# MarineRoboticsGroup/score

Hardware: AMD Instinct MI355X
Metric: socp_iters_per_sec (higher is better)
Workload: dtype f64; 1 GPU; BASELINE configs[3]: manhattan RA-SLAM, 20 robots x 1000 poses, 4 beacons, SOCP relaxation, 1 trial(s)/GPU, ADMM loop alone (polish off) to eps 1e-07; n=146995, m=80979, nnz_P=946147, parallelism=independent x1

## Files before the change

### score_amd/csrc/score_hip.hip

```cpp
#include <hip/hip_runtime.h>
#include <sched.h>
#include <sys/prctl.h>
#include <time.h>
#include <hip/hip_ext.h>

#include <cstdio>
#include <cstring>
#include <malloc.h>
#include <mutex>
#include <string>
#include <memory>
#include <optional>
#include <vector>

#include "score_driver.hpp"
#include <future>
#include "score_assemble.hpp"
#include "score_gn_kernels.hpp"
#include "score_round.hpp"
#include "score_kernels.hpp"
#include "score_polish.hpp"
#include "score_polish_device.hpp"
#include "score_setup_device.hpp"
#include "score_prec_wave.hpp"
// ... 511 lines not shown
        total = 0;
    }
};

inline bool long_spin_enabled() {
    static const bool on = std::getenv("SCORE_NO_LONG_SPIN") == nullptr;
    return on;
}

struct CsrBufs {
    DevBuf<int32_t> ptr, col, first_row, blk_prob, blk_rs, split;
    DevBuf<int4> blk_meta, blk_long;
    DevBuf<double> long_part;
    DevBuf<unsigned long long> long_cnt;
    void alloc_long(int n_long, int n_slots) {
        long_part.alloc((size_t)std::max(1, n_slots) * kLongVals);
        long_cnt.alloc((size_t)std::max(1, n_long));
        fill_zero_async(long_cnt.d, long_cnt.n * sizeof(unsigned long long), tl_copy_stream);
        fill_words_async(long_part.d, (uint32_t)kLongSentinel32, long_part.n * sizeof(double), tl_copy_stream);
    }
    int spin_max_tiles = 0;
    DevBuf<double> val;
    int nblocks = 0;
    int rep = 1;
    int unroll = kUnroll;
    int rs_in = 0;
    void adopt_tiles(const Csr& M, const RowBlocks& rb) {
        UploadBatch ub;
        first_row.upload(rb.first_row);
        blk_prob.upload(rb.prob);
        blk_rs.upload(rb.rs);
// ... 60 lines not shown
        nblocks = L.nb();
        UploadBatch ub;
        V.alloc((size_t)L.v_size + 64);
        fill_zero_async(V.d, V.n * sizeof(double), tl_copy_stream);
        rem_col.upload_padded(L.rem_col, 64);
        rowseg.upload(L.rowseg); dst.upload(L.dst); prob.upload(L.prob); rs.upload(L.rs); part_ptr.upload(L.part_ptr);
        std::vector<int4> m((size_t)nblocks), m2((size_t)nblocks);
        for (int b = 0; b < nblocks; ++b) {
            m[(size_t)b] = make_int4(L.meta[4 * (size_t)b], L.meta[4 * (size_t)b + 1], L.meta[4 * (size_t)b + 2], L.meta[4 * (size_t)b + 3]);
            m2[(size_t)b] = make_int4(L.meta2[4 * (size_t)b], L.meta2[4 * (size_t)b + 1], L.meta2[4 * (size_t)b + 2], L.meta2[4 * (size_t)b + 3]);
        }
        meta.upload(m); meta2.upload(m2);
        std::vector<int4> lg((size_t)nblocks);
        for (int b = 0; b < nblocks; ++b) lg[(size_t)b] = make_int4(L.lng[4 * (size_t)b], L.lng[4 * (size_t)b + 1], L.lng[4 * (size_t)b + 2], L.lng[4 * (size_t)b + 3]);
        lng.upload(lg);
        long_part.alloc((size_t)std::max(1, L.n_long_slots) * kLongVals);
        long_cnt.alloc((size_t)std::max(1, L.n_long));
        fill_zero_async(long_cnt.d, long_cnt.n * sizeof(unsigned long long), tl_copy_stream);
        fill_words_async(long_part.d, (uint32_t)kLongSentinel32, long_part.n * sizeof(double), tl_copy_stream);
    }
    BandDev dev() const {
        BandDev d{};
        d.val = V.d; d.rem_col = rem_col.d; d.rowseg = rowseg.d; d.meta2 = meta2.d; d.rem0 = (int32_t)L.rem0; d.bs = L.bs;
        for (int j = 0; j < kBandMaxS / 2; ++j) d.offw[j] = L.offw[j];
        return d;
    }
};

struct RuizDevice : RuizOffload {
    int device = 0;
    DevArena keep;
// ... 123 lines not shown
        return std::getenv("SCORE_NO_BAND") == nullptr;
    }
    DevBuf<int32_t> A_ptr, A_col;
    DevBuf<double> A_val;
    DevBuf<double> q, b, invD, invE, rho, K0d, K1d;
    DevBuf<int32_t> done, cone_row, cone_dim, cone_type, cone_block_first, cone_block_prob;
    DevBuf<int4> cone_meta;
    DevBuf<int2> cone_large;
    int n_large_cones = 0;
    DevBuf<int32_t> cone_cols;
    DevBuf<double> cone_vals;
    DevBuf<int32_t> node_col, diag_cols, prec_part_ptr;
    DevBuf<PrecWork> prec_work, factor_work;
    DevBuf<int64_t> q_entpart;
    int64_t q_ent_max = 0;
    static constexpr int64_t kHelpEntries = (int64_t)kPrecThreads * kPrecChunk;
    int n_help = 0;
    DevBuf<int32_t> vb_first, vb_end, vb_prob;
    int n_vblocks = 0;
    DevBuf<double> xtu, xy, s, r, z, p, p2, w, kx, step;
    DevBuf<double> pw_part, rz_part0, rz_part1, rz_meas0, rz_meas1, pres_part, dres_part;
    struct GenSource {
        const int32_t* rel_base; const int32_t* rel_to; const double* rel_t; const double* rel_R; const double* rel_kappa; const double* rel_tau;
        const int32_t* rng_a; const int32_t* rng_b; const double* rng_dist; const double* rng_prec;
    };
    const GenSource* gen_src = nullptr;
    int n_join_items = 0, n_join_chains = 0, n_join_seps = 0;
    DevBuf<JoinChain> join_jc;
    DevBuf<JoinItem> join_items;
    DevBuf<int32_t> join_sep_col, join_sep_diag, join_pcol, join_pprev, join_zero;
// ... 775 lines not shown
        }
        set_replica_strides(h);
        upload_cone_tables(h);
        pt.mark("  uploads: cone records");
        {
            UploadBatch ub_tables;
            upload_chain_tables(h);
            plan_split_kernel(h);
        }
        pt.mark("uploads");
        plan_chain_kernel(h);
        const bool polish_from_device = st.polish && init_polish_build(h);
        pt.mark("polish: structure (before the band view is waited for)");
        adopt_band_view(h, pt);
        carve_iterates(h);
        cg_iters = st.cg_iters;
        done.upload(std::vector<int32_t>((size_t)h.count, 0));
        upload_k0_k1(h);
        chain_positions(h);
        join_init(h);
        alloc_factors(h);
        pt.mark("allocations + rho data (device)");
        if (st.polish) init_polish(h, polish_from_device);
        link_init(h, probs, graphs);
        pt.mark("polish setup");
        carve_report_and_control(h);
        reset();
        pt.mark("reset");
        drain_setup();
        pt.mark("staged uploads: drain");
// ... 261 lines not shown
        pl.pre_lds = pl.pre ? lds_pre : 0;
        pl.reg = pl.pre && h.deep_ok && h.bs <= 3 && st.fac_fp32 != 0;
        pl.reg_lds = pl.reg ? lds_reg : 0;
        return pl;
    }
    void plan_chain_kernel(const HostSystem& h) {
        const ChainKernelPlan pl = chain_kernel_plan(h);
        prec_lds0 = pl.lds0; prec_lds = pl.lds;
        prec_pre = pl.pre; prec_pre_lds = pl.pre_lds;
        prec_reg = pl.reg; prec_reg_lds = pl.reg_lds;
        if (prec_reg) deep_map.upload(h.deep_map);
        const bool fallback = !prec_pre || (h.bs >= 4 && st.fac_fp32 == 0);
        if (fallback && prec_lds > 144 * 1024) throw std::runtime_error("chain too long: more than 129 segments of 1023 nodes (132 k) for the segmented chain solver, and beyond what the streaming kernel keeps in LDS");
        if (n_prec_chains(h)) with_bs([&](auto bs) { allow_big_lds<decltype(bs)::value>(); });
    }
    void adopt_band_view(HostSystem& h, PhaseTimer& pt) {
        if (band_job.valid()) {
            Kb.upload(band_job.get());
            if (Kb.on)
                for (int p = 0; p < h.count; ++p) h.kkt_bytes[(size_t)p] = Kb.L.bytes[(size_t)p] + 16.0 * (double)(h.xoff[p + 1] - h.xoff[p]);
            if (st.verbose)
                std::fprintf(stderr, "[score setup] band view of K: %s (%d band + %d csr + %d diag tiles, %d slots per row)\n", Kb.on ? "on" : "off",
                             Kb.L.n_band, Kb.L.n_csr, Kb.L.n_diag, Kb.L.S);
            pt.mark("band view of K (wait + upload)");
        }
        Kset.blk_part.upload(Kb.on ? Kb.L.part_ptr : h.rbK.part_ptr);
    }
    void carve_iterates(const HostSystem& h) {
        const size_t nm = (size_t)(h.n_tot + h.m_tot), nn = (size_t)h.n_tot, mm = (size_t)h.m_tot, cc = (size_t)h.count;
        const size_t kb = (size_t)Kset.blocks(), np_ = (size_t)n_prec;
// ... 625 lines not shown

    SpmvArgs spmv_args(const CsrBufs& M, const double* xin) {
        SpmvArgs a{};
        a.M = M.dev(); a.xin = xin; a.done = done.d; a.rs_in = M.rs_in;
        a.n_tiles = M.nblocks;
        a.x = xy.d; a.q = q.d; a.kx = kx.d; a.r = r.d; a.sigma = H->sigma;
        a.p = p.d; a.w = w.d; a.pw_part = pw_part.d;
        a.prec_part_ptr = prec_part_ptr.d; a.kblk_part_ptr = Kset.blk_part.d;
        a.uni = uni_for(Kset.blocks());
        a.apply_update = 0; a.pfin = p.d; a.wfin = w.d; a.xt_rw = xtu.d; a.kx_rw = kx.d; a.x_rw = xy.d;
        a.alpha_relax = st.alpha; a.step_in = step.d;
        a.invD = invD.d; a.dres_part = dres_part.d;
        return a;
    }

    void launch_kp(const double* pdir, unsigned long long* ts = nullptr, int slot = -1) {
        SpmvArgs a = spmv_args(K, pdir);
        a.p = pdir; a.tstamp = ts;
        launch_product<MODE_KP>(Kset, a, slot);
    }
    void launch_kpb(const double* p_old, double* p_new, const double* rz_new, const double* rz_old,
                    unsigned long long* ts = nullptr, int slot = -1) {
        SpmvArgs a = spmv_args(K, p_old);
        a.tstamp = ts;
        a.p = p_old; a.z = z.d; a.p_out = p_new; a.rz_new = rz_new; a.rz_old = rz_old;
        launch_product<MODE_KPB>(Kset, a, slot);
    }

    void set_cg_iters(int k) {
        cg_iters = std::max(1, k);
        if (graph_exec) { (void)hipGraphExecDestroy(graph_exec); graph_exec = nullptr; }
    }

// ... 10 lines not shown
        }
    }

    VecArgs xupdate_args(const double* p_dir, const double* rz_old, int apply_alpha) {
        VecArgs va{};
        va.first_row = vb_first.d; va.end_row = vb_end.d; va.blk_prob = vb_prob.d; va.done = done.d;
        va.prec_part_ptr = prec_part_ptr.d; va.kblk_part_ptr = Kset.blk_part.d;
        va.pw_part = pw_part.d; va.p = p_dir; va.w = w.d; va.kx = kx.d; va.xt = xtu.d; va.x = xy.d;
        va.alpha_relax = st.alpha; va.rz_old = rz_old; va.apply_alpha = apply_alpha;
        return va;
    }

    size_t ts_stride = 0;
    void enqueue_iteration(bool measure, bool first, unsigned long long* ts = nullptr) {
        auto slot = [&](int k) -> unsigned long long* { return ts ? ts + ts_stride * k : nullptr; };
        {
            SpmvArgs ra = spmv_args(G1, xtu.d);
            ra.tstamp = slot(0);
            ra.apply_update = first ? 0 : 1;
            ra.pfin = last_p;
            launch_spmv<MODE_RHS>(G1, ra, 0);
        }
        PrecArgs pa = prec_args(Kset);
        pa.done = done.d;
        prec_vectors(pa, r.d, r.d, z.d, p.d, w.d, xtu.d, kx.d, pw_part.d);
        double* rz_cur = measure ? rz_meas0.d : rz_part0.d;
        double* p_cur = p.d;
        double* p_oth = p2.d;
        pa.p = p_cur; pa.rz_in = nullptr; pa.rz_out = rz_cur;
        pa.tstamp = slot(1);
        launch_prec<PREC_INIT>(Kset, pa, 1);
        launch_kp(p_cur, slot(2), 2);
        for (int j = 2; j <= cg_iters; ++j) {
            double* rz_nxt = (rz_cur == rz_part0.d) ? rz_part1.d : rz_part0.d;
            pa.p = p_cur; pa.rz_in = rz_cur; pa.rz_out = rz_nxt;
            pa.tstamp = (j == 2) ? slot(3) : nullptr;
            launch_prec<PREC_STEP>(Kset, pa, (j == 2) ? 3 : -1);
            launch_kpb(p_cur, p_oth, rz_nxt, rz_cur, (j == 2) ? slot(4) : nullptr, (j == 2) ? 4 : -1);
            std::swap(p_cur, p_oth);
            rz_cur = rz_nxt;
        }
        dbg_p = p_cur;
        ConeArgs ca = cone_args(xtu.d);
        if (measure) {
            pa.tstamp = nullptr;
            pa.p = p_cur; pa.rz_in = rz_cur; pa.rz_out = rz_meas1.d;
            launch_prec<PREC_STEP>(Kset, pa);
            hipLaunchKernelGGL(k_xupdate, dim3(n_vblocks), dim3(kThreads), 0, stream, xupdate_args(p_cur, rz_cur, 0));
        } else {
            ca.apply_alpha = 1; ca.pfin = p_cur; ca.rz_in = rz_cur;
            last_rz = rz_cur;
            last_p = p_cur;
        }
        ca.tstamp = slot(5);
        if (n_cone_blocks) {
            int chunk = 0;
            const unsigned cgrid = xcd_grid_of(n_cone_blocks, chunk);
            if (chunk) { ca.xcd_chunk = chunk; ca.n_blocks = n_cone_blocks; }
            launch_on_stream(k_cone, dim3(cgrid), dim3(kThreads), 0, 5, ca);
            ca.xcd_chunk = 0;
// ... 1413 lines not shown
```

### score_amd/csrc/score_inspect.hpp

```cpp
#pragma once

struct NewtonProbe {
    static constexpr int kCap = 1024;
    bool armed = false;
    std::vector<hipEvent_t> ev;
    struct Slot { int kind, step; bool real; };
    std::vector<Slot> slots;
    size_t marked = 0;
    double out[8] = {0, 0, 0, 0, 0, 0, 0, 0};
};
int probe_slot(HipBackend& be, int kind, int step) {
    NewtonProbe* np = be.probe.get();
    if (!np || !np->armed || (int)np->slots.size() >= NewtonProbe::kCap) return -1;
    np->slots.push_back(NewtonProbe::Slot{kind, step, false});
    be.tev = np->ev.data();
    return (int)np->slots.size() - 1;
}
void probe_mark(HipBackend& be, int used) {
    NewtonProbe* np = be.probe.get();
    if (!np) return;
    for (; np->marked < np->slots.size(); ++np->marked)
        if (np->slots[np->marked].step < used) np->slots[np->marked].real = true;
}
void probe_collect(HipBackend& be) {
// ... 101 lines not shown
    return copy_out_min(v, 3, out, len);
}
int64_t get_links(HipBackend& be, double* out, int64_t len) {
    double v[6] = {(double)be.link_plan.pairs_total, (double)be.link_plan.pairs_used, (double)be.n_link_u, (double)be.n_link_items, (double)be.link_rounds, 0.0};
    if (be.n_link_probs && out) {
        std::vector<int32_t> stt((size_t)be.n_link_probs);
        HIP_CHECK(sync_stream(be.stream));
        for (int set = 0; set < 2; ++set) {
            if (!be.pset[set].link_on) continue;
            HIP_CHECK(hipMemcpy(stt.data(), be.pset[set].link_status.d, sizeof(int32_t) * (size_t)be.n_link_probs, hipMemcpyDeviceToHost));
            for (int32_t x : stt) v[5] += x;
        }
    }
    return copy_out_min(v, 6, out, len);
}
int64_t get_newton_probe(HipBackend& be, double* out, int64_t len) {
    static const double none[8] = {0, 0, 0, 0, 0, 0, 0, 0};
    return copy_out_min(be.probe ? be.probe->out : none, 8, out, len);
}
double mismatches(const std::vector<int32_t>& x, const std::vector<int32_t>& y) {
    double c = (double)(x.size() > y.size() ? x.size() - y.size() : y.size() - x.size());
    for (size_t i = 0; i < std::min(x.size(), y.size()); ++i) c += x[i] != y[i];
    return c;
}
double max_diff(const std::vector<double>& x, const std::vector<double>& y) {
    double c = x.size() == y.size() ? 0.0 : 1e300;
    for (size_t i = 0; i < std::min(x.size(), y.size()); ++i) c = std::max(c, std::fabs(x[i] - y[i]));
    return c;
}
int64_t get_ag_device_check(HipBackend& be, double* out, int64_t len) {
// ... 105 lines not shown
        {"is_head", ds ? R::DevI32 : R::HostI32, ds ? (const void*)be.q_ishead.d : Q.is_head.data(), ds ? n : (int64_t)Q.is_head.size(), polish},
        {"Hcol", be.polish_on_device ? R::DevI32 : R::HostI32, be.polish_on_device ? (const void*)be.Hm.col.d : Q.Hm.col.data(),
         be.polish_on_device ? be.hm_nnz : (int64_t)Q.Hm.col.size(), polish},
        {"Hptr", R::HostI32, Q.Hm.ptr.data(), (int64_t)Q.Hm.ptr.size(), polish},
        {"link_pairs", R::HostI32, be.link_plan.pair_cols.data(), be.n_link_items ? (int64_t)be.link_plan.pair_cols.size() : 0},
    };
    for (const R& r : rows)
        if (nm == r.name) return read_row(be, r, out, len);
    struct Computed { const char* name; int64_t (*fn)(HipBackend&, double*, int64_t); };
    static const Computed computed[] = {
        {"setup_scalars", get_setup_scalars}, {"device_setup", get_device_setup}, {"rep", get_rep}, {"links", get_links},
        {"newton_probe_arm", probe_arm}, {"newton_probe", get_newton_probe}, {"ag_device_check", get_ag_device_check},
        {"polish_build_check", get_polish_build_check}, {"polish_assemble_at_x", get_polish_assemble_at_x},
        {"polish_prec_of_negg", get_polish_prec_of_negg},
        {"chain_of_col", get_chain_of_col}, {"chain_id_of_col", get_chain_id_of_col}, {"matrix_source", get_matrix_source},
    };
    for (const Computed& c : computed)
        if (nm == c.name) return c.fn(be, out, len);
    return -1;
}

struct TimeAllActive {
    HipBackend& be;
    std::vector<int32_t> keep;
    explicit TimeAllActive(HipBackend& b) : be(b), keep((size_t)b.H->count) {
        const std::vector<int32_t> zero(keep.size(), 0);
        HIP_CHECK(sync_stream(be.stream));
        HIP_CHECK(hipMemcpyAsync(keep.data(), be.done.d, keep.size() * sizeof(int32_t), hipMemcpyDeviceToHost, be.stream));
        HIP_CHECK(sync_stream(be.stream));
        HIP_CHECK(hipMemcpyAsync(be.done.d, zero.data(), zero.size() * sizeof(int32_t), hipMemcpyHostToDevice, be.stream));
// ... 128 lines not shown
```

### score_amd/csrc/score_kernels.hpp

```cpp
#pragma once

#include <type_traits>

#include <hip/hip_runtime.h>

#include "score_host.hpp"
#include "score_band.hpp"

namespace score {

#ifdef SCORE_NT_STORES
#define NTS(lhs, val) __builtin_nontemporal_store((val), &(lhs))
#else
#define NTS(lhs, val) ((lhs) = (val))
#endif
#if defined(SCORE_NT_STORES) || defined(SCORE_NT_PREC)
#define NTSP(lhs, val) __builtin_nontemporal_store((val), &(lhs))
#else
#define NTSP(lhs, val) ((lhs) = (val))
#endif

constexpr int kThreads = 256;
constexpr int kUnroll = kTileNnz / kThreads;
constexpr int kLongUnroll = 2;
constexpr int kPartStride = 12;

__device__ __forceinline__ double wave_sum(double v) {
#pragma unroll
    for (int off = 32; off > 0; off >>= 1) v += __shfl_down(v, off, 64);
    return v;
}
__device__ __forceinline__ double wave_max(double v) {
#pragma unroll
    for (int off = 32; off > 0; off >>= 1) v = fmax(v, __shfl_down(v, off, 64));
    return v;
}
__device__ __forceinline__ double block_sum(double v, double* red) {
    v = wave_sum(v);
    __syncthreads();
    if ((threadIdx.x & 63) == 0) red[threadIdx.x >> 6] = v;
// ... 53 lines not shown

struct CsrDev {
    const int32_t* ptr;
    const int32_t* col;
    const double* val;
    const int32_t* first_row;
    const int32_t* blk_prob;
    const int4* blk_meta;
    const int32_t* blk_rs;
    const int32_t* split;
    int nblocks;
    const int4* blk_long;
    double* long_part;
    unsigned long long* long_cnt;
    int long_spin;
};
constexpr unsigned long long kLongSentinel = 0x7ff8dead7ff8deadull;
constexpr unsigned kLongSentinel32 = 0x7ff8deadu;

struct KernelStamp {
    unsigned long long* ts;
    __device__ explicit KernelStamp(unsigned long long* p) : ts(p) {
        if (ts && threadIdx.x == 0) ts[2 * blockIdx.x] = (unsigned long long)wall_clock64();
    }
    __device__ ~KernelStamp() {
        if (ts && threadIdx.x == 0) ts[2 * blockIdx.x + 1] = (unsigned long long)wall_clock64();
    }
};

struct UniRanges {
    int on;
    int l0, l1;
    int k0, k1;
};

struct BandDev {
    const double* val;
    const int32_t* rem_col;
    const int32_t* rowseg;
    const int4* meta2;
    int32_t rem0;
    int32_t bs;
    int32_t offw[kBandMaxS / 2];
};

struct SpmvArgs {
    UniRanges uni;
    CsrDev M;
    BandDev B;
// ... 22 lines not shown
    double* xt_rw;
    double* kx_rw;
    double* x_rw;
    double alpha_relax;
    const double* step_in;
    const int32_t* kblk_part_ptr;
    const int32_t* is_head;
    double* gout;
    const double* invD;
    double* dres_part;
    unsigned long long* tstamp;
};

enum { MODE_RHS = 0, MODE_KP = 1, MODE_DRES = 2, MODE_KPB = 3, MODE_GRAD = 4 };

constexpr int kMaxRep = 3;

__device__ __forceinline__ void soc_scales(int type, double t0, double nz2, double& head, double& tail) {
    if (type == 0) {
        head = 0.0; tail = 0.0;
        return;
    }
    const double nz = sqrt(nz2);
    if (nz <= t0) { head = t0; tail = 1.0; }
    else if (nz <= -t0) { head = 0.0; tail = 0.0; }
    else { const double m = 0.5 * (t0 + nz); head = m; tail = m / nz; }
}

struct TileHead {
    int4 meta, m2, lg;
    int prob, rs, dn0;
};
// ... 45 lines not shown
        if (MODE == MODE_KPB) {
            if (pi0 < pl1) { acc_n = a.rz_new[pi0]; acc_o = a.rz_old[pi0]; }
            for (int i = pi0 + kThreads; i < pl1; i += kThreads) { acc_n += a.rz_new[i]; acc_o += a.rz_old[i]; }
        }
    };
    if (MODE == MODE_RHS && a.apply_update) beta = a.step_in[prob];
    auto finish_beta = [&]() {
        if (MODE == MODE_KPB) {
            block_sum2(acc_n, acc_o, red);
            beta = acc_o > 0.0 ? acc_n / acc_o : 0.0;
        }
    };

    int row = r0 + t;
    bool has_row = false;
    double sum[NR], sum2 = 0.0;
#pragma unroll
    for (int q = 0; q < NR; ++q) sum[q] = 0.0;
    const int dn = a.uni.on ? dn0 : a.done[prob];
    const int my_ptr = a.M.ptr[min(r0 + t, r1)];
    const int nseg = lg.y & 0xffff;
    const bool one_long = (r1 - r0 == 1 && (nn > kLongRow || nseg > 1));
    int b = b_in;
    const int ro = one_long ? r0 : min(row, max(r1 - 1, r0));
    double e0[NR], e1[NR], e2[NR], e3[NR], e4[NR], e5[NR];
#pragma unroll
    for (int q = 0; q < NR; ++q) {
        const int o = ro + q * rs_out;
        e0[q] = e1[q] = e2[q] = e3[q] = e4[q] = e5[q] = 0.0;
        if (MODE == MODE_RHS) {
// ... 62 lines not shown
                    if ((MODE == MODE_DRES || MODE == MODE_GRAD) && k >= split) acc2 += pr; else acc[q] += pr;
                }
            }
        }
        if (MODE == MODE_DRES || MODE == MODE_GRAD) {
            block_sum2(acc[0], acc2, red);
            sum[0] = acc[0]; sum2 = acc2;
        } else if (NR == 1) {
            sum[0] = block_sum(acc[0], red);
        } else {
            block_sum2(acc[0], acc[1], red);
            sum[0] = acc[0]; sum[1] = acc[1];
            if (NR > 2) sum[NR - 1] = block_sum(acc[NR - 1], red);
        }
        const bool spin = nseg > 1 && a.M.long_spin && nseg * kLongVals <= NR * kPlane;
        if (spin) {
            constexpr int NV = NR + ((MODE == MODE_DRES || MODE == MODE_GRAD) ? 1 : 0);
            const int sgi = lg.y >> 16;
            unsigned long long* allb = reinterpret_cast<unsigned long long*>(a.M.long_part + (size_t)lg.z * kLongVals);
            if (sgi != 0) {
                if (t == 0) {
                    unsigned long long* slot = allb + (size_t)sgi * kLongVals;
#pragma unroll
                    for (int q = 0; q < NR; ++q) __hip_atomic_store(slot + q, (unsigned long long)__double_as_longlong(sum[q]), __ATOMIC_RELAXED, __HIP_MEMORY_SCOPE_AGENT);
                    if (MODE == MODE_DRES || MODE == MODE_GRAD)
                        __hip_atomic_store(slot + NR, (unsigned long long)__double_as_longlong(sum2), __ATOMIC_RELAXED, __HIP_MEMORY_SCOPE_AGENT);
                }
                return;
            }
            const int total = nseg * kLongVals;
            int ok = 0;
// ... 129 lines not shown
    if (MODE == MODE_RHS) {
        if (has_row) {
#pragma unroll
            for (int q = 0; q < NR; ++q) {
                const int o = row + q * rs_out;
                double kxv = e0[q];
                double xv = e1[q];
                if (a.apply_update) {
                    const double xt = e3[q] + beta * e4[q];
                    kxv += beta * e5[q];
                    xv = a.alpha_relax * xt + (1.0 - a.alpha_relax) * xv;
                    NTS(a.xt_rw[o], xt);
                    NTS(a.kx_rw[o], kxv);
                    NTS(a.x_rw[o], xv);
                }
                NTS(a.r[o], a.sigma * xv - e2[q] + sum[q] - kxv);
            }
        }
    } else if (MODE == MODE_KP || MODE == MODE_KPB) {
        double local = 0.0;
        if (has_row) {
#pragma unroll
            for (int q = 0; q < NR; ++q) {
                const int o = row + q * rs_out;
                double pi, sq = sum[q];
                if (MODE == MODE_KPB) {
                    sq += beta * e0[q];
                    pi = e1[q] + beta * e2[q];
                    NTS(a.p_out[o], pi);
                } else {
                    pi = e0[q];
// ... 352 lines not shown
struct PrecArgs {
    const PrecWork* work;
    const PrecRecord* rec;
    const ChainDesc* chains;
    const ChainLevelDesc* levels;
    const double* fac;
    const float* fac32;
    const float* deep;
    const int32_t* node_col;
    const int32_t* diag_cols;
    const double* dinv;
    const int32_t* done;
    const int32_t* prec_part_ptr;
    const int32_t* kblk_part_ptr;
    UniRanges uni;
    double* r;
    double* z;
    double* p;
    const double* w;
    double* xt;
    double* kx;
    const double* rz_in;
    const double* pw_part;
    double* rz_out;
    unsigned long long* tstamp;
    int debug_skip;
    int n_vec;
    long long vec_stride;
    int split_update;
    const double* r_in;
// ... 55 lines not shown
    const size_t eP = (size_t)L.P * L.nruns;
    const double* __restrict__ R = fac + L.offR;
#pragma unroll
    for (int q = 0; q < RMAX; ++q) {
        const double* __restrict__ Rq = R + (size_t)min(q, len - 1) * L.nruns + j;
#pragma unroll
        for (int e = 0; e < B2; ++e) {
            Lf[q][e] = Rq[(size_t)e * eP];
            Dv[q][e] = Rq[(size_t)(B2 + e) * eP];
        }
    }
}

template <int MODE>
__device__ __forceinline__ double prec_jacobi_item(const PrecArgs& a, const PrecWork& wk, double acc_rz, double acc_pw,
                                                   double* red, bool& stop) {
    const int t = threadIdx.x;
    double alpha = 0.0, local = 0.0;
    stop = false;
    if (MODE == PREC_STEP) {
        const double gref = (a.gate_flag && !a.gate_first) ? a.gate_ref[wk.prob] : 0.0;
        block_sum2_n<kPrecWaves>(acc_rz, acc_pw, red);
        alpha = acc_pw > 0.0 ? acc_rz / acc_pw : 0.0;
        if (pcg_gate(a, wk.prob, acc_rz, gref)) { stop = true; return 0.0; }
    }
    const int e_end = wk.index + wk.count;
    for (int base = wk.index + t; base < e_end; base += kPrecThreads * kPrecChunk) {
        int cols[kPrecChunk];
        double rv[kPrecChunk], dv[kPrecChunk], pv[kPrecChunk], wv[kPrecChunk], xv[kPrecChunk], kv[kPrecChunk];
#pragma unroll
        for (int u = 0; u < kPrecChunk; ++u) cols[u] = a.diag_cols[min(base + u * kPrecThreads, e_end - 1)];
#pragma unroll
        for (int u = 0; u < kPrecChunk; ++u) {
            rv[u] = a.r_in[cols[u]];
            dv[u] = a.dinv[min(base + u * kPrecThreads, e_end - 1)];
            if (MODE == PREC_STEP) {
                wv[u] = a.w[cols[u]];
                if (!a.split_update) { pv[u] = a.p[cols[u]]; xv[u] = a.xt_zero ? 0.0 : a.xt[cols[u]]; kv[u] = a.kx[cols[u]]; }
                else { pv[u] = 0.0; xv[u] = 0.0; kv[u] = 0.0; }
            }
        }
#pragma unroll
        for (int u = 0; u < kPrecChunk; ++u) {
            if (base + u * kPrecThreads < e_end) {
                double r_ = rv[u];
                if (MODE == PREC_STEP) {
                    if (!a.split_update) {
                        NTSP(a.xt[cols[u]], xv[u] + alpha * pv[u]);
                        NTSP(a.kx[cols[u]], kv[u] + alpha * wv[u]);
                    }
                    r_ -= alpha * wv[u];
                    NTSP(a.r[cols[u]], r_);
                }
                const double zv = r_ * dv[u];
                NTSP(a.z[cols[u]], zv);
                if (MODE == PREC_INIT) NTSP(a.p[cols[u]], zv);
                local += r_ * zv;
            }
        }
    }
    return local;
}

__device__ __forceinline__ void prec_select_vector(PrecArgs& a) {
    if (a.n_vec > 1) {
        const long long off = (long long)blockIdx.y * a.vec_stride;
// ... 334 lines not shown
    constexpr int B2 = BS * BS;
    constexpr int oRun = REGDEEP ? 2 * B2 : 0;
    constexpr int oBk2 = 10 * B2;
    constexpr int NG = REGDEEP ? 12 * B2 : PreTile<BS>::NG;
    constexpr int oCl = oRun + 2 * RMAX * B2, oCr = oCl + B2;
    constexpr int kStageLanes = kPrecThreads - kPreRunLanes;
    constexpr int CH = PreTile<BS>::CH;
    using LT = typename std::conditional<(BS >= 4 || REGDEEP), FT, double>::type;
    extern __shared__ __attribute__((aligned(16))) double lds[];
    __shared__ PrecRecord srec;
    double* red = lds;
    const int t = threadIdx.x;
    double acc_rz = 0.0, acc_pw = 0.0;
    int4 rec4 = make_int4(0, 0, 0, 0);
    if (t < 32) rec4 = reinterpret_cast<const int4*>(a.rec + blockIdx.x)[t];
    const int dn0 = a.uni.on ? a.done[0] : 0;
    if (MODE == PREC_STEP && a.uni.on) {
        const int i0 = a.uni.l0 + t, j0 = a.uni.k0 + t;
        if (i0 < a.uni.l1) acc_rz = a.rz_in[i0];
        if (j0 < a.uni.k1) acc_pw = a.pw_part[j0];
        for (int i = i0 + kPrecThreads; i < a.uni.l1; i += kPrecThreads) acc_rz += a.rz_in[i];
        for (int i = j0 + kPrecThreads; i < a.uni.k1; i += kPrecThreads) acc_pw += a.pw_part[i];
    }
    if (t < 32) reinterpret_cast<int4*>(&srec)[t] = rec4;
    __syncthreads();
    const PrecWork wk = srec.wk;
    const ChainLevelDesc* sLv = srec.lv;
    const int prob = wk.prob;
    const int dn_ld = a.uni.on ? dn0 : a.done[prob];
    int bl0 = 0, bl1 = 0, bk0 = 0, bk1 = 0;
    if (MODE == PREC_STEP && !a.uni.on) {
        bl0 = a.prec_part_ptr[prob]; bl1 = a.prec_part_ptr[prob + 1];
        bk0 = a.kblk_part_ptr[prob]; bk1 = a.kblk_part_ptr[prob + 1];
    }
    int dn = 0;
    if (a.early_done) {
        dn = dn_ld;
        if (dn) return;
    }
    const int dn_late = a.early_done ? 0 : dn_ld;
    if (MODE == PREC_INIT && a.gate_init && threadIdx.x == 0 && (int)blockIdx.x == a.prec_part_ptr[prob]) {
        a.gate_init[prob] = a.early_done ? dn : dn_late;
        a.gate_used[prob] = 0;
// ... 6 lines not shown
        for (int i = k0 + t + kPrecThreads; i < k1; i += kPrecThreads) acc_pw += a.pw_part[i];
    }
    double local = 0.0;
    if (wk.kind == 2) {
        if (dn || dn_late) return;
        if (MODE == PREC_INIT) return;
        const double gref = (a.gate_flag && !a.gate_first) ? a.gate_ref[prob] : 0.0;
        const int e_end = wk.index + wk.count;
        int idx[kPrecChunk];
        double pv[kPrecChunk], wv[kPrecChunk], xv[kPrecChunk], kv[kPrecChunk];
#pragma unroll
        for (int u = 0; u < kPrecChunk; ++u) {
            idx[u] = min(wk.index + t + u * kPrecThreads, e_end - 1);
            pv[u] = a.p[idx[u]]; wv[u] = a.w[idx[u]]; xv[u] = a.xt_zero ? 0.0 : a.xt[idx[u]]; kv[u] = a.kx[idx[u]];
        }
        block_sum2_n<kPrecWaves>(acc_rz, acc_pw, red);
        const double alpha = acc_pw > 0.0 ? acc_rz / acc_pw : 0.0;
        if (a.gate_flag && (a.gate_first ? !(acc_rz > 0.0) : !(acc_rz > gref))) return;
#pragma unroll
        for (int u = 0; u < kPrecChunk; ++u) {
            if (wk.index + t + u * kPrecThreads < e_end) {
                NTSP(a.xt[idx[u]], xv[u] + alpha * pv[u]);
                NTSP(a.kx[idx[u]], kv[u] + alpha * wv[u]);
            }
        }
        return;
    }
    if (wk.kind == 1) {
        if (dn || dn_late) return;
        bool stop;
        local = prec_jacobi_item<MODE>(a, wk, acc_rz, acc_pw, red, stop);
        if (stop) return;
    } else {
        const double gref = (MODE == PREC_STEP && a.gate_flag && !a.gate_first) ? a.gate_ref[prob] : 0.0;
        const ChainDesc ch = srec.ch;
        const FT* __restrict__ fac = sizeof(FT) == 4 ? (const FT*)(const void*)a.fac32 : (const FT*)(const void*)a.fac;
        const int N = ch.N;
        const int NB = N * BS;
        const int nl = ch.n_levels;
        const int stride = ch.col_stride, col0 = ch.col0;
        auto colof = [&](int node) -> int { return col0 + node * stride; };
        double* vb = lds + 16;
        double* v0 = vb;
        const ChainLevelDesc L0 = sLv[0];
        const ChainLevelDesc Lz = sLv[nl - 1];
        LT* lfac = reinterpret_cast<LT*>(vb + Lz.lds_off + Lz.N * BS + 1);
// ... 863 lines not shown
```

Before: 17720 iters/s.

## Defer long-row split partial sums to the next preconditioner kernel instead of spinning

For SpMV rows split across several tiles (long rows), the RHS and KP kernels now write per-segment partials to a second slot region and exit, instead of spin-waiting on counters for the other segments to finish. The following preconditioner kernel loads these partials into shared memory, finishes the reductions for the few affected Jacobi columns, fixes up w/r and the p·Kp partial, and writes the final values. The goal is to remove the inter-workgroup spin synchronization from the critical path. In exchange, the long-partial buffer doubles in size, the preconditioner kernel does extra lookups, and the path applies only in a narrow single-problem configuration.

```diff
diff --git a/score_amd/csrc/score_hip.hip b/score_amd/csrc/score_hip.hip
--- a/score_amd/csrc/score_hip.hip
+++ b/score_amd/csrc/score_hip.hip
@@ -1,3 +1,5 @@
+#include <array>
+#include <climits>
 #include <hip/hip_runtime.h>
 #include <sched.h>
 #include <sys/prctl.h>
@@ -549,7 +551,7 @@
     DevBuf<double> long_part;
     DevBuf<unsigned long long> long_cnt;
     void alloc_long(int n_long, int n_slots) {
-        long_part.alloc((size_t)std::max(1, n_slots) * kLongVals);
+        long_part.alloc((size_t)2 * std::max(1, n_slots) * kLongVals);
         long_cnt.alloc((size_t)std::max(1, n_long));
         fill_zero_async(long_cnt.d, long_cnt.n * sizeof(unsigned long long), tl_copy_stream);
         fill_words_async(long_part.d, (uint32_t)kLongSentinel32, long_part.n * sizeof(double), tl_copy_stream);
@@ -640,7 +642,7 @@
         std::vector<int4> lg((size_t)nblocks);
         for (int b = 0; b < nblocks; ++b) lg[(size_t)b] = make_int4(L.lng[4 * (size_t)b], L.lng[4 * (size_t)b + 1], L.lng[4 * (size_t)b + 2], L.lng[4 * (size_t)b + 3]);
         lng.upload(lg);
-        long_part.alloc((size_t)std::max(1, L.n_long_slots) * kLongVals);
+        long_part.alloc((size_t)2 * std::max(1, L.n_long_slots) * kLongVals);
         long_cnt.alloc((size_t)std::max(1, L.n_long));
         fill_zero_async(long_cnt.d, long_cnt.n * sizeof(unsigned long long), tl_copy_stream);
         fill_words_async(long_part.d, (uint32_t)kLongSentinel32, long_part.n * sizeof(double), tl_copy_stream);
@@ -794,6 +796,13 @@
     DevBuf<PrecWork> prec_work, factor_work;
     DevBuf<int64_t> q_entpart;
     int64_t q_ent_max = 0;
+    struct DeferPlan {
+        LongDefer tab{};
+        int offset = 0;
+        int split_rows = 0;
+    };
+    DeferPlan defer_kp, defer_rhs;
+    bool long_defer_enabled = true;
     static constexpr int64_t kHelpEntries = (int64_t)kPrecThreads * kPrecChunk;
     int n_help = 0;
     DevBuf<int32_t> vb_first, vb_end, vb_prob;
@@ -1599,6 +1608,7 @@
         pt.mark("polish: structure (before the band view is waited for)");
         adopt_band_view(h, pt);
         carve_iterates(h);
+        plan_long_defer(h);
         cg_iters = st.cg_iters;
         done.upload(std::vector<int32_t>((size_t)h.count, 0));
         upload_k0_k1(h);
@@ -1890,6 +1900,70 @@
         if (fallback && prec_lds > 144 * 1024) throw std::runtime_error("chain too long: more than 129 segments of 1023 nodes (132 k) for the segmented chain solver, and beyond what the streaming kernel keeps in LDS");
         if (n_prec_chains(h)) with_bs([&](auto bs) { allow_big_lds<decltype(bs)::value>(); });
     }
+    template <class Tile>
+    DeferPlan plan_defer_rows(const HostSystem& h, int nb, int n_slots, bool polls, double* part, Tile&& tile) const {
+        DeferPlan P;
+        for (int b = 0; b < nb; ++b) {
+            const std::array<int32_t, 5> tl = tile(b);
+            if ((tl[2] & 0xffff) > 1 && (tl[2] >> 16) == 0) ++P.split_rows;
+        }
+        const bool single = h.count == 1 && active_part_ptr.size() == 2 && !split.active;
+        if (!single || !polls || P.split_rows == 0 || P.split_rows > kDeferRows || n_slots * kLongVals > kDeferVals ||
+            Kset.blocks() > kPrecThreads)
+            return P;
+        std::vector<char> jacobi((size_t)h.n_tot, 0);
+        for (const PrecWork& wk : h.prec_work)
+            if (wk.kind == 1)
+                for (int32_t e = wk.index; e < wk.index + wk.count; ++e) jacobi[(size_t)h.diag_cols[(size_t)e]] = 1;
+        LongDefer d{};
+        d.lo = INT32_MAX; d.hi = -1;
+        for (int b = 0; b < nb; ++b) {
+            const std::array<int32_t, 5> tl = tile(b);
+            const int nseg = tl[2] & 0xffff;
+            if (nseg <= 1 || (tl[2] >> 16) != 0) continue;
+            const int nr = tl[1] > 0 ? h.rep : 1;
+            for (int k = 0; k < nr; ++k) {
+                const int64_t idx = (int64_t)tl[0] + (int64_t)k * tl[1];
+                if (idx < 0 || idx >= h.n_tot || !jacobi[(size_t)idx]) return P;
+                d.lo = std::min<int>(d.lo, (int)idx); d.hi = std::max<int>(d.hi, (int)idx);
+            }
+            if (tl[3] < 0 || tl[3] + nseg > n_slots) return P;
+            d.col[d.n] = tl[0]; d.rs[d.n] = tl[1]; d.nr[d.n] = nr; d.slot[d.n] = tl[3]; d.nseg[d.n] = nseg; d.pw[d.n] = tl[4];
+            ++d.n;
+        }
+        d.n_vals = n_slots * kLongVals;
+        d.part = part + (size_t)n_slots * kLongVals;
+        P.tab = d;
+        P.offset = n_slots;
+        return P;
+    }
+    void plan_long_defer(const HostSystem& h) {
+        const bool spin = long_spin_enabled();
+        if (Kb.on) {
+            const BandLayout& L = Kb.L;
+            defer_kp = plan_defer_rows(h, Kb.nblocks, L.n_long_slots, spin && Kb.nblocks <= K.spin_max_tiles, Kb.long_part.d, [&L](int b) {
+                const size_t i = 4 * (size_t)b;
+                return std::array<int32_t, 5>{L.meta[i], L.rs[(size_t)b], L.lng[i + 1], L.lng[i + 2], L.lng[i]};
+            });
+        } else {
+            const RowBlocks& rb = h.rbK;
+            defer_kp = plan_defer_rows(h, K.nblocks, rb.n_long_slots, spin && K.nblocks <= K.spin_max_tiles, K.long_part.d, [&rb](int b) {
+                return std::array<int32_t, 5>{rb.first_row[(size_t)b], rb.rs[(size_t)b], rb.lseg[(size_t)b], rb.lbase[(size_t)b], rb.lfirst[(size_t)b]};
+            });
+        }
+        defer_kp.tab.w_out = w.d;
+        const RowBlocks& rg = h.rbG1;
+        defer_rhs = plan_defer_rows(h, G1.nblocks, rg.n_long_slots, spin && G1.nblocks <= G1.spin_max_tiles, G1.long_part.d, [&rg](int b) {
+            return std::array<int32_t, 5>{rg.first_row[(size_t)b], rg.rs[(size_t)b], rg.lseg[(size_t)b], rg.lbase[(size_t)b], rg.lfirst[(size_t)b]};
+        });
+        defer_rhs.tab.x = xy.d; defer_rhs.tab.q = q.d; defer_rhs.tab.sigma = h.sigma;
+    }
+    bool chain_is_pre(const PrecSet& S) const { return !split.active && S.rec.d != nullptr && prec_pre && (H->bs <= 3 || S.use_fac32); }
+    const DeferPlan* defer_for(const DeferPlan& P, bool kp) const {
+        const bool on = long_defer_enabled && P.offset > 0 && chain_is_pre(Kset) && (!kp || cg_iters >= 2);
+        return on ? &P : nullptr;
+    }
+
     void adopt_band_view(HostSystem& h, PhaseTimer& pt) {
         if (band_job.valid()) {
             Kb.upload(band_job.get());
@@ -2545,9 +2619,9 @@
         return a;
     }
 
-    void launch_kp(const double* pdir, unsigned long long* ts = nullptr, int slot = -1) {
+    void launch_kp(const double* pdir, unsigned long long* ts = nullptr, int slot = -1, int long_defer = 0) {
         SpmvArgs a = spmv_args(K, pdir);
-        a.p = pdir; a.tstamp = ts;
+        a.p = pdir; a.tstamp = ts; a.M.long_defer = long_defer;
         launch_product<MODE_KP>(Kset, a, slot);
     }
     void launch_kpb(const double* p_old, double* p_new, const double* rz_new, const double* rz_old,
@@ -2588,11 +2662,14 @@
     size_t ts_stride = 0;
     void enqueue_iteration(bool measure, bool first, unsigned long long* ts = nullptr) {
         auto slot = [&](int k) -> unsigned long long* { return ts ? ts + ts_stride * k : nullptr; };
+        const DeferPlan* d_rhs = defer_for(defer_rhs, false);
+        const DeferPlan* d_kp = defer_for(defer_kp, true);
         {
             SpmvArgs ra = spmv_args(G1, xtu.d);
             ra.tstamp = slot(0);
             ra.apply_update = first ? 0 : 1;
             ra.pfin = last_p;
+            if (d_rhs) ra.M.long_defer = d_rhs->offset;
             launch_spmv<MODE_RHS>(G1, ra, 0);
         }
         PrecArgs pa = prec_args(Kset);
@@ -2603,12 +2680,15 @@
         double* p_oth = p2.d;
         pa.p = p_cur; pa.rz_in = nullptr; pa.rz_out = rz_cur;
         pa.tstamp = slot(1);
+        if (d_rhs) pa.defer = d_rhs->tab;
         launch_prec<PREC_INIT>(Kset, pa, 1);
-        launch_kp(p_cur, slot(2), 2);
+        pa.defer = LongDefer{};
+        launch_kp(p_cur, slot(2), 2, d_kp ? d_kp->offset : 0);
         for (int j = 2; j <= cg_iters; ++j) {
             double* rz_nxt = (rz_cur == rz_part0.d) ? rz_part1.d : rz_part0.d;
             pa.p = p_cur; pa.rz_in = rz_cur; pa.rz_out = rz_nxt;
             pa.tstamp = (j == 2) ? slot(3) : nullptr;
+            pa.defer = (j == 2 && d_kp) ? d_kp->tab : LongDefer{};
             launch_prec<PREC_STEP>(Kset, pa, (j == 2) ? 3 : -1);
             launch_kpb(p_cur, p_oth, rz_nxt, rz_cur, (j == 2) ? slot(4) : nullptr, (j == 2) ? 4 : -1);
             std::swap(p_cur, p_oth);
@@ -2618,6 +2698,7 @@
         ConeArgs ca = cone_args(xtu.d);
         if (measure) {
             pa.tstamp = nullptr;
+            pa.defer = LongDefer{};
             pa.p = p_cur; pa.rz_in = rz_cur; pa.rz_out = rz_meas1.d;
             launch_prec<PREC_STEP>(Kset, pa);
             hipLaunchKernelGGL(k_xupdate, dim3(n_vblocks), dim3(kThreads), 0, stream, xupdate_args(p_cur, rz_cur, 0));
diff --git a/score_amd/csrc/score_inspect.hpp b/score_amd/csrc/score_inspect.hpp
--- a/score_amd/csrc/score_inspect.hpp
+++ b/score_amd/csrc/score_inspect.hpp
@@ -139,6 +139,47 @@
     }
     return copy_out_min(v, 6, out, len);
 }
+int64_t get_long_defer(HipBackend& be, double* out, int64_t len) {
+    auto most = [](const RowBlocks* rb, const BandLayout* L) {
+        int m = 0;
+        if (L) { for (size_t i = 1; i < L->lng.size(); i += 4) m = std::max(m, L->lng[i] & 0xffff); }
+        else { for (int32_t v : rb->lseg) m = std::max(m, v & 0xffff); }
+        return (double)m;
+    };
+    const HipBackend::DeferPlan* dk = be.defer_for(be.defer_kp, true);
+    const HipBackend::DeferPlan* dr = be.defer_for(be.defer_rhs, false);
+    const double v[7] = {dk ? (double)dk->tab.n : 0.0, dr ? (double)dr->tab.n : 0.0, (double)be.defer_kp.split_rows, (double)be.defer_rhs.split_rows,
+                         most(&be.H->rbK, be.Kb.on ? &be.Kb.L : nullptr), most(&be.H->rbG1, nullptr), be.chain_is_pre(be.Kset) ? 1.0 : 0.0};
+    return copy_out_min(v, 7, out, len);
+}
+int64_t get_long_tiles(HipBackend& be, double* out, int64_t len) {
+    std::vector<double> v;
+    auto add = [&](int which, int nb, auto&& lng) {
+        int chunk = 0;
+        (void)HipBackend::xcd_grid_of(nb, chunk);
+        for (int b = 0; b < nb; ++b) {
+            const std::array<int32_t, 2> lg = lng(b);
+            if ((lg[0] & 0xffff) <= 1) continue;
+            const int wg = chunk ? (b % chunk) * 8 + b / chunk : b;
+            v.insert(v.end(), {(double)which, (double)wg, (double)lg[1], (double)(lg[0] >> 16)});
+        }
+    };
+    if (be.Kb.on) { const BandLayout& L = be.Kb.L; add(0, be.Kb.nblocks, [&L](int b) { return std::array<int32_t, 2>{L.lng[4 * (size_t)b + 1], L.lng[4 * (size_t)b + 3]}; }); }
+    else { const RowBlocks& rb = be.H->rbK; add(0, be.K.nblocks, [&rb](int b) { return std::array<int32_t, 2>{rb.lseg[(size_t)b], rb.lid[(size_t)b]}; }); }
+    const RowBlocks& rg = be.H->rbG1;
+    add(1, be.G1.nblocks, [&rg](int b) { return std::array<int32_t, 2>{rg.lseg[(size_t)b], rg.lid[(size_t)b]}; });
+    return copy_out_min(v.data(), (int64_t)v.size(), out, len);
+}
+int64_t set_long_defer(HipBackend& be, bool on, double* out, int64_t len) {
+    if (out && len > 0) {
+        be.long_defer_enabled = on;
+        if (be.graph_exec) { (void)hipGraphExecDestroy(be.graph_exec); be.graph_exec = nullptr; }
+    }
+    const double v = on ? 1.0 : 0.0;
+    return copy_out_min(&v, 1, out, len);
+}
+int64_t long_defer_off(HipBackend& be, double* out, int64_t len) { return set_long_defer(be, false, out, len); }
+int64_t long_defer_on(HipBackend& be, double* out, int64_t len) { return set_long_defer(be, true, out, len); }
 int64_t get_newton_probe(HipBackend& be, double* out, int64_t len) {
     static const double none[8] = {0, 0, 0, 0, 0, 0, 0, 0};
     return copy_out_min(be.probe ? be.probe->out : none, 8, out, len);
@@ -274,6 +315,7 @@
         {"polish_build_check", get_polish_build_check}, {"polish_assemble_at_x", get_polish_assemble_at_x},
         {"polish_prec_of_negg", get_polish_prec_of_negg},
         {"chain_of_col", get_chain_of_col}, {"chain_id_of_col", get_chain_id_of_col}, {"matrix_source", get_matrix_source},
+        {"long_defer", get_long_defer}, {"long_tiles", get_long_tiles}, {"long_defer_off", long_defer_off}, {"long_defer_on", long_defer_on},
     };
     for (const Computed& c : computed)
         if (nm == c.name) return c.fn(be, out, len);
diff --git a/score_amd/csrc/score_kernels.hpp b/score_amd/csrc/score_kernels.hpp
--- a/score_amd/csrc/score_kernels.hpp
+++ b/score_amd/csrc/score_kernels.hpp
@@ -24,6 +24,7 @@
 constexpr int kUnroll = kTileNnz / kThreads;
 constexpr int kLongUnroll = 2;
 constexpr int kPartStride = 12;
+constexpr int kMaxRep = 3;
 
 __device__ __forceinline__ double wave_sum(double v) {
 #pragma unroll
@@ -107,6 +108,7 @@
     double* long_part;
     unsigned long long* long_cnt;
     int long_spin;
+    int long_defer;
 };
 constexpr unsigned long long kLongSentinel = 0x7ff8dead7ff8deadull;
 constexpr unsigned kLongSentinel32 = 0x7ff8deadu;
@@ -126,6 +128,43 @@
     int l0, l1;
     int k0, k1;
 };
+
+constexpr int kDeferRows = 8;
+constexpr int kDeferVals = 128;
+struct LongDefer {
+    int n;
+    int n_vals;
+    int lo, hi;
+    const double* part;
+    int col[kDeferRows];
+    int rs[kDeferRows];
+    int nr[kDeferRows];
+    int slot[kDeferRows];
+    int nseg[kDeferRows];
+    int pw[kDeferRows];
+    double* w_out;
+    const double* x;
+    const double* q;
+    double sigma;
+};
+__device__ __forceinline__ double long_defer_sum(const double* sdef, const int slot, const int nseg, const int q) {
+    double tot = 0.0;
+    for (int sg = 0; sg < nseg; ++sg) tot += sdef[(slot + sg) * kLongVals + q];
+    return tot;
+}
+__device__ __forceinline__ bool long_defer_find(const LongDefer& d, const int idx, int& slot, int& nseg, int& q) {
+    bool hit = false;
+    slot = 0; nseg = 0; q = 0;
+#pragma unroll
+    for (int j = 0; j < kDeferRows; ++j) {
+        if (j < d.n) {
+#pragma unroll
+            for (int k = 0; k < kMaxRep; ++k)
+                if (k < d.nr[j] && idx == d.col[j] + k * d.rs[j]) { hit = true; slot = d.slot[j]; nseg = d.nseg[j]; q = k; }
+        }
+    }
+    return hit;
+}
 
 struct BandDev {
     const double* val;
@@ -178,8 +217,6 @@
 
 enum { MODE_RHS = 0, MODE_KP = 1, MODE_DRES = 2, MODE_KPB = 3, MODE_GRAD = 4 };
 
-constexpr int kMaxRep = 3;
-
 __device__ __forceinline__ void soc_scales(int type, double t0, double nz2, double& head, double& tail) {
     if (type == 0) {
         head = 0.0; tail = 0.0;
@@ -255,6 +292,7 @@
 
     int row = r0 + t;
     bool has_row = false;
+    bool deferred = false;
     double sum[NR], sum2 = 0.0;
 #pragma unroll
     for (int q = 0; q < NR; ++q) sum[q] = 0.0;
@@ -347,7 +385,20 @@
             if (NR > 2) sum[NR - 1] = block_sum(acc[NR - 1], red);
         }
         const bool spin = nseg > 1 && a.M.long_spin && nseg * kLongVals <= NR * kPlane;
-        if (spin) {
+        if ((MODE == MODE_KP || MODE == MODE_RHS) && nseg > 1 && a.M.long_defer > 0) {
+            const int sgi = lg.y >> 16;
+            if (t == 0) {
+                double* slot = a.M.long_part + (size_t)(a.M.long_defer + lg.z + sgi) * kLongVals;
+#pragma unroll
+                for (int q = 0; q < NR; ++q) slot[q] = sum[q];
+            }
+            if (sgi != 0) return;
+            if (MODE == MODE_KP) {
+                for (int i = t; i < nseg; i += kThreads) a.pw_part[lg.x + i] = 0.0;
+                return;
+            }
+            deferred = true;
+        } else if (spin) {
             constexpr int NV = NR + ((MODE == MODE_DRES || MODE == MODE_GRAD) ? 1 : 0);
             const int sgi = lg.y >> 16;
             unsigned long long* allb = reinterpret_cast<unsigned long long*>(a.M.long_part + (size_t)lg.z * kLongVals);
@@ -507,7 +558,7 @@
                     NTS(a.kx_rw[o], kxv);
                     NTS(a.x_rw[o], xv);
                 }
-                NTS(a.r[o], a.sigma * xv - e2[q] + sum[q] - kxv);
+                if (!deferred) NTS(a.r[o], a.sigma * xv - e2[q] + sum[q] - kxv);
             }
         }
     } else if (MODE == MODE_KP || MODE == MODE_KPB) {
@@ -890,6 +941,7 @@
     const int32_t* prec_part_ptr;
     const int32_t* kblk_part_ptr;
     UniRanges uni;
+    LongDefer defer;
     double* r;
     double* z;
     double* p;
@@ -975,7 +1027,7 @@
 
 template <int MODE>
 __device__ __forceinline__ double prec_jacobi_item(const PrecArgs& a, const PrecWork& wk, double acc_rz, double acc_pw,
-                                                   double* red, bool& stop) {
+                                                   double* red, bool& stop, const double* sdef = nullptr) {
     const int t = threadIdx.x;
     double alpha = 0.0, local = 0.0;
     stop = false;
@@ -986,8 +1038,10 @@
         if (pcg_gate(a, wk.prob, acc_rz, gref)) { stop = true; return 0.0; }
     }
     const int e_end = wk.index + wk.count;
+    const bool defer = sdef != nullptr && a.defer.n > 0;
     for (int base = wk.index + t; base < e_end; base += kPrecThreads * kPrecChunk) {
         int cols[kPrecChunk];
+        bool dfr[kPrecChunk];
         double rv[kPrecChunk], dv[kPrecChunk], pv[kPrecChunk], wv[kPrecChunk], xv[kPrecChunk], kv[kPrecChunk];
 #pragma unroll
         for (int u = 0; u < kPrecChunk; ++u) cols[u] = a.diag_cols[min(base + u * kPrecThreads, e_end - 1)];
@@ -999,6 +1053,20 @@
                 wv[u] = a.w[cols[u]];
                 if (!a.split_update) { pv[u] = a.p[cols[u]]; xv[u] = a.xt_zero ? 0.0 : a.xt[cols[u]]; kv[u] = a.kx[cols[u]]; }
                 else { pv[u] = 0.0; xv[u] = 0.0; kv[u] = 0.0; }
+            }
+            dfr[u] = false;
+            if (defer) {
+                int sl, ns, q;
+                if (long_defer_find(a.defer, cols[u], sl, ns, q)) {
+                    const double fin = long_defer_sum(sdef, sl, ns, q);
+                    dfr[u] = true;
+                    if (MODE == PREC_STEP) {
+                        wv[u] = fin;
+                    } else {
+                        const double xq = a.defer.x[cols[u]], qq = a.defer.q[cols[u]], kxq = a.kx[cols[u]];
+                        rv[u] = a.defer.sigma * xq - qq + fin - kxq;
+                    }
+                }
             }
         }
 #pragma unroll
@@ -1011,6 +1079,9 @@
                         NTSP(a.kx[cols[u]], kv[u] + alpha * wv[u]);
                     }
                     r_ -= alpha * wv[u];
+                    NTSP(a.r[cols[u]], r_);
+                    if (dfr[u]) NTSP(a.defer.w_out[cols[u]], wv[u]);
+                } else if (dfr[u]) {
                     NTSP(a.r[cols[u]], r_);
                 }
                 const double zv = r_ * dv[u];
@@ -1375,6 +1446,24 @@
     double acc_rz = 0.0, acc_pw = 0.0;
     int4 rec4 = make_int4(0, 0, 0, 0);
     if (t < 32) rec4 = reinterpret_cast<const int4*>(a.rec + blockIdx.x)[t];
+    __shared__ double sdef[kDeferVals];
+    const bool dfr_on = a.defer.n > 0;
+    double dslot = 0.0, dp[kMaxRep] = {0.0, 0.0, 0.0};
+    int d_slot = 0, d_nseg = 0, d_nr = 0;
+    bool d_mine = false;
+    if (dfr_on) {
+        if (t < a.defer.n_vals) dslot = a.defer.part[t];
+        if (MODE == PREC_STEP) {
+            int d_col = 0, d_rs = 0;
+#pragma unroll
+            for (int j = 0; j < kDeferRows; ++j)
+                if (j < a.defer.n && a.uni.k0 + t == a.defer.pw[j]) {
+                    d_mine = true; d_col = a.defer.col[j]; d_rs = a.defer.rs[j]; d_nr = a.defer.nr[j]; d_slot = a.defer.slot[j]; d_nseg = a.defer.nseg[j];
+                }
+#pragma unroll
+            for (int q = 0; q < kMaxRep; ++q) dp[q] = a.p[d_col + (q < d_nr ? q : 0) * d_rs];
+        }
+    }
     const int dn0 = a.uni.on ? a.done[0] : 0;
     if (MODE == PREC_STEP && a.uni.on) {
         const int i0 = a.uni.l0 + t, j0 = a.uni.k0 + t;
@@ -1384,10 +1473,21 @@
         for (int i = j0 + kPrecThreads; i < a.uni.k1; i += kPrecThreads) acc_pw += a.pw_part[i];
     }
     if (t < 32) reinterpret_cast<int4*>(&srec)[t] = rec4;
+    if (dfr_on && t < a.defer.n_vals) sdef[t] = dslot;
     __syncthreads();
     const PrecWork wk = srec.wk;
     const ChainLevelDesc* sLv = srec.lv;
     const int prob = wk.prob;
+    if (MODE == PREC_STEP && d_mine) {
+        double local = 0.0;
+#pragma unroll
+        for (int q = 0; q < kMaxRep; ++q)
+            if (q < d_nr) {
+                const double sq = long_defer_sum(sdef, d_slot, d_nseg, q);
+                local += dp[q] * sq;
+            }
+        acc_pw = local;
+    }
     const int dn_ld = a.uni.on ? dn0 : a.done[prob];
     int bl0 = 0, bl1 = 0, bk0 = 0, bk1 = 0;
     if (MODE == PREC_STEP && !a.uni.on) {
@@ -1424,6 +1524,13 @@
             idx[u] = min(wk.index + t + u * kPrecThreads, e_end - 1);
             pv[u] = a.p[idx[u]]; wv[u] = a.w[idx[u]]; xv[u] = a.xt_zero ? 0.0 : a.xt[idx[u]]; kv[u] = a.kx[idx[u]];
         }
+        if (dfr_on && wk.index <= a.defer.hi && e_end > a.defer.lo) {
+#pragma unroll
+            for (int u = 0; u < kPrecChunk; ++u) {
+                int sl, ns, q;
+                if (long_defer_find(a.defer, idx[u], sl, ns, q)) wv[u] = long_defer_sum(sdef, sl, ns, q);
+            }
+        }
         block_sum2_n<kPrecWaves>(acc_rz, acc_pw, red);
         const double alpha = acc_pw > 0.0 ? acc_rz / acc_pw : 0.0;
         if (a.gate_flag && (a.gate_first ? !(acc_rz > 0.0) : !(acc_rz > gref))) return;
@@ -1439,7 +1546,7 @@
     if (wk.kind == 1) {
         if (dn || dn_late) return;
         bool stop;
-        local = prec_jacobi_item<MODE>(a, wk, acc_rz, acc_pw, red, stop);
+        local = prec_jacobi_item<MODE>(a, wk, acc_rz, acc_pw, red, stop, sdef);
         if (stop) return;
     } else {
         const double gref = (MODE == PREC_STEP && a.gate_flag && !a.gate_first) ? a.gate_ref[prob] : 0.0;
```

Measured after the change: 17080 iters/s. 3.6% lower.
